# socom20/speech-cloner

Measured on AMD Instinct MI355X. Metric: mel frames/sec, higher is better.
Workload: dtype bf16; 1 GPU; full: STFT+mel front-end on batch 32 x 4 s @ 16 kHz (configs[1] input) -> 64 windows of 400 frames -> encoder (enc_14 weights) + decoder (hp/decoder_cfg_d.json sizes, random init), 64 windows per launch, independent steps pipelined over 10 HIP streams; batch=32, samples=64000, windows=64, model_dtype=bfloat16, streams=10, parallelism=utterance-sharded x1, no collective

## Files before the change

speech-cloner_amd/csrc/vc_common.h:

```cpp
#pragma once
#include <hip/hip_runtime.h>
#include <cstdarg>
#include <cstdio>
#include "vc_hip.h"

namespace vc {

char* last_error_buf();
int set_error(int code, const char* fmt, ...);

#define VC_HIP_CHECK(expr)                                                                   \
    do {                                                                                     \
        hipError_t _e = (expr);                                                              \
        if (_e != hipSuccess)                                                                \
            return vc::set_error(VC_ERR_HIP, "%s failed: %s (%s:%d)", #expr,                 \
                                 hipGetErrorString(_e), __FILE__, __LINE__);                 \
    } while (0)

#define VC_REQUIRE(cond, ...)                                                                \
    do {                                                                                     \
        if (!(cond)) return vc::set_error(VC_ERR_INVALID, __VA_ARGS__);                      \
    } while (0)

constexpr int WAVE = 64;

enum Option {
    OPT_BANK256 = 0,
    OPT_BANK256_XCD,
    OPT_CONV256,
    OPT_CONV256_MINK,
    OPT_CONV256_WM,
    OPT_PROJ256,
    OPT_PROJ256_SPLIT,
    OPT_WGRAD_XCD,
    OPT_GRU_MFMA,
    OPT_FE_FUSED,
    OPT_FE_FUSED_SPIN,
    OPT_PRENET_LDS,
    OPT_GRU_TRAIN_RESIDENT,
    OPT_CBHG_FRONT_MI,
    OPT_GRU_F32_WIDE,
    OPT_F32_F16X3,
    OPT_GEMM16_SPLIT,
    OPT_COUNT
};
int opt(Option o);

hipError_t zero_async(void* d_p, size_t bytes, hipStream_t st);

#if defined(__HIPCC__)
template <int CTRL, int ROW_MASK>
__device__ __forceinline__ float dpp_move(float identity, float v) {
    return __int_as_float(__builtin_amdgcn_update_dpp(__float_as_int(identity), __float_as_int(v), CTRL, ROW_MASK, 0xF, false));
}
#define VC_WAVE_REDUCE(OP, ID)                                                                  \
    v = OP(v, dpp_move<0xB1, 0xF>(ID, v));                             \
    v = OP(v, dpp_move<0x4E, 0xF>(ID, v));                             \
    v = OP(v, dpp_move<0x141, 0xF>(ID, v));                                \
    v = OP(v, dpp_move<0x140, 0xF>(ID, v));          \
    v = OP(v, dpp_move<0x142, 0xA>(ID, v));                 \
    v = OP(v, dpp_move<0x143, 0xC>(ID, v));                 \
    return __int_as_float(__builtin_amdgcn_readlane(__float_as_int(v), 63));
__device__ __forceinline__ float vc_addf(float a, float b) { return a + b; }
__device__ __forceinline__ float wave_sum(float v) { VC_WAVE_REDUCE(vc_addf, 0.0f) }
__device__ __forceinline__ float wave_max(float v) { VC_WAVE_REDUCE(fmaxf, -3.402823466e38f) }
__device__ __forceinline__ float wave_max_inf(float v) { VC_WAVE_REDUCE(fmaxf, v) }
__device__ __forceinline__ float highway_gate(float hpre, float tpre, float x) {
    const float hv = fmaxf(hpre, 0.0f);
    const float e = __builtin_amdgcn_exp2f(tpre * -1.4426950408889634f);
    const float tv = __builtin_amdgcn_rcpf(1.0f + e);
    return fmaf(tv, hv - x, x);
}
__device__ __forceinline__ float wave_min(float v) { VC_WAVE_REDUCE(fminf, 3.402823466e38f) }
#undef VC_WAVE_REDUCE
struct ArgMax { float v; int idx; };
__device__ __forceinline__ ArgMax wave_argmax_low(float v, int idx) {
#pragma unroll
    for (int s = 32; s > 0; s >>= 1) {
        const float ov = __shfl_xor(v, s, 64);
        const int oi = __shfl_xor(idx, s, 64);
        if (ov > v || (ov == v && oi < idx)) { v = ov; idx = oi; }
    }
    return {v, idx};
}

template <bool SUM, int NW>
__device__ inline int block_scan_excl(int v, int* wtot, int& total) {
    const int lane = threadIdx.x & 63, wave = threadIdx.x >> 6;
    const int ident = SUM ? 0 : -1;
    int inc = v;
#pragma unroll
    for (int s = 1; s < 64; s <<= 1) {
        const int u = __shfl_up(inc, s, 64);
        if (lane >= s) inc = SUM ? inc + u : max(inc, u);
    }
    int excl = __shfl_up(inc, 1, 64);
    if (lane == 0) excl = ident;
    __syncthreads();
    if (lane == 63) wtot[wave] = inc;
    __syncthreads();
    int off = ident, all = ident;
    for (int w = 0; w < NW; ++w) {
        const int x = wtot[w];
        if (w < wave) off = SUM ? off + x : max(off, x);
        all = SUM ? all + x : max(all, x);
    }
    total = all;
    return SUM ? excl + off : max(excl, off);
}

__device__ __forceinline__ float power_db_to_amp(float P, float inv_norm) {
    return exp10f(0.05f * (fmaxf(0.0f, P) * inv_norm - 80.0f));
}
#endif

}
```

speech-cloner_amd/csrc/vc_gemm.hip:

```cpp
#include <hip/hip_runtime.h>

#include <cstdlib>
#include "vc_device.h"
#include "vc_bank256.h"
#include "vc_conv256.h"

using vc::f32x16, vc::f32x4, vc::bf16x8;

namespace {

constexpr int BN = 128;
constexpr int ROWB = 144;
constexpr int GEMM_THREADS = 256;
constexpr int lds_bytes(int MI) { return 2 * (64 * MI + BN) * ROWB; }

template <typename T> struct Tr;
template <> struct Tr<float> {
    static constexpr int VEC = 4, BK = 32;
    typedef f32x4 vec_t;
};
template <> struct Tr<__bf16> {
    static constexpr int VEC = 8, BK = 64;
    typedef bf16x8 vec_t;
};
// ... 15 lines not shown
    const void* R;
    int32_t ldr;
    void* C;
    int32_t ldc, out_f32;
    float drop_keep;
    unsigned long long drop_seed;
    int32_t sum_groups;
    KGroup g[VC_GEMM_MAX_GROUPS];
};

__device__ __forceinline__ bool drop_keep_elem(unsigned long long idx, unsigned long long seed, float keep) {
    unsigned long long x = idx + seed * 0x9E3779B97F4A7C15ull;
    x ^= x >> 30; x *= 0xBF58476D1CE4E5B9ull;
    x ^= x >> 27; x *= 0x94D049BB133111EBull;
    x ^= x >> 31;
    return (float)(unsigned)(x >> 40) < keep * 16777216.0f;
}

__device__ __forceinline__ float to_f32(float v) { return v; }
__device__ __forceinline__ float to_f32(__bf16 v) { return (float)v; }

template <typename T> __device__ __forceinline__ void store_out(void* C, size_t idx, float v, int out_f32) {
    if (out_f32) reinterpret_cast<float*>(C)[idx] = v;
    else reinterpret_cast<T*>(C)[idx] = (T)v;
}

__device__ __forceinline__ f32x4 pro_apply(f32x4 v, const float* sc, const float* sh, int c, int relu) {
#pragma unroll
    for (int e = 0; e < 4; ++e) {
        float x = v[e];
        if (sc) x = x * sc[c + e] + sh[c + e];
        if (relu) x = fmaxf(x, 0.0f);
        v[e] = x;
    }
    return v;
}
__device__ __forceinline__ bf16x8 pro_apply(bf16x8 v, const float* sc, const float* sh, int c, int relu) {
#pragma unroll
    for (int e = 0; e < 8; ++e) {
        float x = (float)v[e];
        if (sc) x = x * sc[c + e] + sh[c + e];
        if (relu) x = fmaxf(x, 0.0f);
        v[e] = (__bf16)x;
    }
    return v;
}
__device__ __forceinline__ f32x4 vmax(f32x4 a, f32x4 b) {
#pragma unroll
    for (int e = 0; e < 4; ++e) a[e] = fmaxf(a[e], b[e]);
    return a;
}
__device__ __forceinline__ bf16x8 vmax(bf16x8 a, bf16x8 b) {
#pragma unroll
    for (int e = 0; e < 8; ++e) a[e] = ((float)a[e] >= (float)b[e]) ? a[e] : b[e];
    return a;
}

template <typename T, int MI> struct Mma;

template <int MI> struct Mma<float, MI> {
    static __device__ __forceinline__ void slab(const char* As, const char* Bs, int wm, int wn, int lane,
                                                f32x16 (&acc)[MI][2]) {
        const int i = lane & 31, h = lane >> 5;
        const char* ap = As + (wm * 32 * MI + i) * ROWB + h * 16;
        const char* bp = Bs + (wn * 64 + i) * ROWB + h * 16;
#pragma unroll
        for (int p = 0; p < 4; ++p) {
            f32x4 av[MI], bv[2];
#pragma unroll
            for (int mi = 0; mi < MI; ++mi) av[mi] = *reinterpret_cast<const f32x4*>(ap + mi * 32 * ROWB + p * 32);
            bv[0] = *reinterpret_cast<const f32x4*>(bp + p * 32);
            bv[1] = *reinterpret_cast<const f32x4*>(bp + 32 * ROWB + p * 32);
#pragma unroll
            for (int q = 0; q < 4; ++q)
#pragma unroll
                for (int mi = 0; mi < MI; ++mi)
#pragma unroll
                    for (int ni = 0; ni < 2; ++ni)
                        acc[mi][ni] = __builtin_amdgcn_mfma_f32_32x32x2f32(av[mi][q], bv[ni][q], acc[mi][ni], 0, 0, 0);
        }
    }
};

template <int MI> struct Mma<__bf16, MI> {
    static __device__ __forceinline__ void slab(const char* As, const char* Bs, int wm, int wn, int lane,
                                                f32x16 (&acc)[MI][2]) {
        const int i = lane & 31, h = lane >> 5;
        const char* ap = As + (wm * 32 * MI + i) * ROWB + h * 16;
        const char* bp = Bs + (wn * 64 + i) * ROWB + h * 16;
#pragma unroll
        for (int s = 0; s < 4; ++s) {
            bf16x8 av[MI], bv[2];
#pragma unroll
            for (int mi = 0; mi < MI; ++mi) av[mi] = *reinterpret_cast<const bf16x8*>(ap + mi * 32 * ROWB + s * 32);
            bv[0] = *reinterpret_cast<const bf16x8*>(bp + s * 32);
            bv[1] = *reinterpret_cast<const bf16x8*>(bp + 32 * ROWB + s * 32);
#pragma unroll
            for (int mi = 0; mi < MI; ++mi)
#pragma unroll
                for (int ni = 0; ni < 2; ++ni)
                    acc[mi][ni] = __builtin_amdgcn_mfma_f32_32x32x16_bf16(av[mi], bv[ni], acc[mi][ni], 0, 0, 0);
        }
    }
};


struct EpiCoef { float s[2], b[2]; };
__device__ __forceinline__ EpiCoef epilogue_coef(const KArgs& a, const KGroup& grp, int n0, int wn, int lane) {
    EpiCoef c;
#pragma unroll
    for (int ni = 0; ni < 2; ++ni) {
        const int oc = grp.c_off + min(n0 + wn * 64 + ni * 32 + (lane & 31), a.N - 1);
        c.s[ni] = a.epi_scale ? a.epi_scale[oc] : 1.0f;
        c.b[ni] = a.epi_shift ? a.epi_shift[oc] : 0.0f;
    }
    return c;
}

template <typename T, int MI>
__device__ __forceinline__ void epilogue_tile(const KArgs& a, const KGroup& grp, char* smem, const f32x16 (&acc)[MI][2],
                                              const EpiCoef& coef, int m0, int n0, int row_w, int wn, int lane, int tid) {
    constexpr int BM = 64 * MI;
    const bool f32o = a.out_f32 || sizeof(T) == 4;
    const int es = f32o ? 4 : 2;
    const int pitch = 128 * es + 16;
    const int i = lane & 31, h = lane >> 5;
#pragma unroll
    for (int ni = 0; ni < 2; ++ni) {
        const int lcol = wn * 64 + ni * 32 + i;
        const int gn = min(n0 + lcol, a.N - 1);
        const int oc = grp.c_off + gn;
        const float s = coef.s[ni], b = coef.b[ni];
#pragma unroll
        for (int mi = 0; mi < MI; ++mi) {
#pragma unroll
            for (int r = 0; r < 16; ++r) {
                const int lrow = row_w + mi * 32 + (r & 3) + 8 * (r >> 2) + 4 * h;
                const int gm = min(m0 + lrow, a.M - 1);
                float v = vc::act_fn(acc[mi][ni][r] * s + b, a.act);
                if (a.drop_keep > 0.0f)
                    v = drop_keep_elem((unsigned long long)gm * a.ldc + oc, a.drop_seed, a.drop_keep) ? v / a.drop_keep : 0.0f;
                if (a.R) v += to_f32(reinterpret_cast<const T*>(a.R)[(size_t)gm * a.ldr + gn]);
                char* dst = smem + lrow * pitch + lcol * es;
                if (f32o) *reinterpret_cast<float*>(dst) = v;
                else *reinterpret_cast<__bf16*>(dst) = (__bf16)v;
            }
        }
    }
    __syncthreads();
    const int chunk = 16 / es;
    const int cpr = 128 / chunk;
    char* C = reinterpret_cast<char*>(a.C);
    const bool vec_ok = ((reinterpret_cast<uintptr_t>(C) & 15) == 0) && ((a.ldc * es) % 16 == 0) &&
                        (((grp.c_off + n0) * es) % 16 == 0);
    for (int idx = tid; idx < BM * cpr; idx += GEMM_THREADS) {
        const int row = idx / cpr, ch = idx - row * cpr;
        const int gm = m0 + row, gn0 = n0 + ch * chunk;
        if (gm >= a.M || gn0 >= a.N) continue;
        const char* src = smem + row * pitch + ch * 16;
        char* dst = C + ((size_t)gm * a.ldc + grp.c_off + gn0) * es;
        if (vec_ok && gn0 + chunk <= a.N) {
            *reinterpret_cast<f32x4*>(dst) = *reinterpret_cast<const f32x4*>(src);
        } else {
            const int n = min(chunk, a.N - gn0);
            for (int e = 0; e < n; ++e) {
                if (f32o) reinterpret_cast<float*>(dst)[e] = reinterpret_cast<const float*>(src)[e];
                else reinterpret_cast<unsigned short*>(dst)[e] = reinterpret_cast<const unsigned short*>(src)[e];
            }
        }
    }
}

template <typename T, int MODE, int MI, int PRO>
__global__ void __launch_bounds__(GEMM_THREADS, 2)
gemm_kernel(KArgs a) {
    typedef typename Tr<T>::vec_t vec_t;
    constexpr int VEC = Tr<T>::VEC, BK = Tr<T>::BK;
    constexpr int BM = 64 * MI, AP = 2 * MI;
    constexpr int A_BYTES = BM * ROWB, B_BYTES = BN * ROWB, BUF_BYTES = A_BYTES + B_BYTES;
    extern __shared__ __attribute__((aligned(16))) char smem[];

    const int tid = threadIdx.x, lane = tid & 63, wid = tid >> 6;
    const int wm = wid >> 1, wn = wid & 1;
    const KGroup grp = a.g[a.n_groups - 1 - (int)blockIdx.y];
    const int ntn = (a.N + BN - 1) / BN;
    const int mt = blockIdx.x / ntn, nt = blockIdx.x - mt * ntn;
    const int m0 = mt * BM, n0 = nt * BN;
    const int K = grp.K, Cin = a.Cin, Tn = a.T;
    const int nk = (K + BK - 1) / BK;
    const T* X = reinterpret_cast<const T*>(a.X);
    const T* Bt = reinterpret_cast<const T*>(grp.Bt);

    const int sc = tid & 7, sr = tid >> 3;
    const T* a_row[AP];
    int a_t[AP];
    bool a_ok[AP], b_ok[4];
    const T* b_row[4];
#pragma unroll
    for (int p = 0; p < AP; ++p) {
        const int m = m0 + sr + 32 * p;
        a_ok[p] = m < a.M;
        const int mm = min(m, a.M - 1);
        a_t[p] = mm % Tn;
        a_row[p] = X + (size_t)mm * a.ldx;
    }
#pragma unroll
    for (int p = 0; p < 4; ++p) {
        const int n = n0 + sr + 32 * p;
        b_ok[p] = n < a.N;
        b_row[p] = Bt + (size_t)min(n, a.N - 1) * K;
    }
    const int pad_l = grp.pad_l, ldx = a.ldx;
    const bool pool = PRO >= 1 && a.pro_pool != 0;
    const bool nonneg = a.pro_pool == 2 || a.pro_relu;

    vec_t ra[AP], ra2[PRO >= 1 ? AP : 1], rb[4];
    unsigned okbits = 0;
    int st_c = 0;
    int g_kk = sc * VEC, g_j = 0, g_c = sc * VEC;
    if (grp.taps > 1) { g_j = g_c / Cin; g_c -= g_j * Cin; }
    auto gload = [&]() {
        const bool kok = g_kk < K;
        const int j = kok ? g_j : 0, c = kok ? g_c : 0, kb = kok ? g_kk : 0;
        const int dj = j - pad_l;
        unsigned bits = 0;
#pragma unroll
        for (int p = 0; p < AP; ++p) {
            const int tt = a_t[p] + dj;
            const bool ok = kok && a_ok[p] && tt >= 0 && tt < Tn;
            const T* ptr = a_row[p] + (ok ? dj * ldx : 0) + c;
            ra[p] = *reinterpret_cast<const vec_t*>(ptr);
            if (PRO >= 1) {
                const T* ptr2 = ptr + ((pool && ok && tt + 1 < Tn) ? ldx : 0);
                ra2[p] = *reinterpret_cast<const vec_t*>(ptr2);
            }
            bits |= (ok ? 1u : 0u) << p;
        }
#pragma unroll
        for (int p = 0; p < 4; ++p) {
            rb[p] = *reinterpret_cast<const vec_t*>(b_row[p] + kb);
            bits |= ((kok && b_ok[p]) ? 1u : 0u) << (8 + p);
        }
        okbits = bits;
        st_c = c;
        g_kk += BK;
        g_c += BK;
        if (grp.taps > 1)
            while (g_c >= Cin) { g_c -= Cin; ++g_j; }
    };
    auto lstore = [&](int buf) {
        char* As = smem + buf * BUF_BYTES;
        char* Bs = As + A_BYTES;
        const vec_t zero = {};
#pragma unroll
        for (int p = 0; p < AP; ++p) {
            vec_t v = ra[p];
            if (PRO == 2) v = pro_apply(v, a.pro_scale, a.pro_shift, st_c, a.pro_relu);
            if (PRO >= 1) {
                vec_t v2 = ra2[p];
                if (PRO == 2) v2 = pro_apply(v2, a.pro_scale, a.pro_shift, st_c, a.pro_relu);
                if (pool) v = nonneg ? vc::max_nonneg(v, v2) : vmax(v, v2);
            }
            *reinterpret_cast<vec_t*>(As + (sr + 32 * p) * ROWB + sc * 16) = ((okbits >> p) & 1u) ? v : zero;
        }
#pragma unroll
        for (int p = 0; p < 4; ++p)
            *reinterpret_cast<vec_t*>(Bs + (sr + 32 * p) * ROWB + sc * 16) = ((okbits >> (8 + p)) & 1u) ? rb[p] : zero;
    };

    f32x16 acc[MI][2];
#pragma unroll
    for (int mi = 0; mi < MI; ++mi)
#pragma unroll
        for (int ni = 0; ni < 2; ++ni)
#pragma unroll
            for (int r = 0; r < 16; ++r) acc[mi][ni][r] = 0.0f;

    const EpiCoef coef = (MODE == VC_GEMM_PLAIN) ? epilogue_coef(a, grp, n0, wn, lane) : EpiCoef{};
    gload();
    lstore(0);
    __syncthreads();
    for (int kt = 0; kt < nk; ++kt) {
        const bool more = kt + 1 < nk;
        if (more) gload();
        const char* As = smem + (kt & 1) * BUF_BYTES;
        Mma<T, MI>::slab(As, As + A_BYTES, wm, wn, lane, acc);
        if (more) lstore((kt + 1) & 1);
        __syncthreads();
    }

    const int i = lane & 31, h = lane >> 5;
    if (MODE == VC_GEMM_PLAIN) {
        epilogue_tile<T, MI>(a, grp, smem, acc, coef, m0, n0, wm * 32 * MI, wn, lane, tid);
    } else {
        const int hc = (n0 + wn * 64) / 2 + i;
        const int Hn = Cin;
        if (hc < Hn) {
            const int gnH = n0 + wn * 64 + i, gnT = gnH + 32;
            const float bH = a.epi_shift ? a.epi_shift[gnH] : 0.0f;
            const float bT = a.epi_shift ? a.epi_shift[gnT] : 0.0f;
#pragma unroll
            for (int mi = 0; mi < MI; ++mi) {
#pragma unroll
                for (int r = 0; r < 16; ++r) {
                    const int gm = m0 + wm * 32 * MI + mi * 32 + (r & 3) + 8 * (r >> 2) + 4 * h;
                    if (gm >= a.M) continue;
                    const float xv = to_f32(X[(size_t)gm * a.ldx + hc]);
                    store_out<T>(a.C, (size_t)gm * a.ldc + hc, vc::highway_gate(acc[mi][0][r] + bH, acc[mi][1][r] + bT, xv), a.out_f32);
                }
            }
        }
    }
}


constexpr int CONV_MAX_TAPS = 32;
constexpr int CROWB = ROWB;
constexpr int conv_lds_bytes() {
    return (128 + CONV_MAX_TAPS - 1) * CROWB + 2 * BN * CROWB > 128 * 528 ? (128 + CONV_MAX_TAPS - 1) * CROWB + 2 * BN * CROWB : 128 * 528;
}
__device__ __forceinline__ int swz(int row, int chunk) { return row * CROWB + (chunk << 4); }

template <typename T, int PRO>
__global__ void __launch_bounds__(GEMM_THREADS, 2)
conv_kernel(KArgs a) {
    typedef typename Tr<T>::vec_t vec_t;
    constexpr int VEC = Tr<T>::VEC, BK = Tr<T>::BK;
    constexpr int BM = 128, MI = 2;
    constexpr int A_BYTES = (BM + CONV_MAX_TAPS - 1) * CROWB, B_BYTES = BN * CROWB;
    constexpr int NAP = 5;
    extern __shared__ __attribute__((aligned(16))) char smem[];
    char* const As = smem;
    char* const Bs0 = smem + A_BYTES;

    const int tid = threadIdx.x, lane = tid & 63, wid = tid >> 6;
    const int wm = wid >> 1, wn = wid & 1;
    const int ntn = (a.N + BN - 1) / BN;
    const int mt = blockIdx.x / ntn, nt = blockIdx.x - mt * ntn;
    const int m0 = mt * BM, n0 = nt * BN;
    const int Cin = a.Cin, Tn = a.T, ldx = a.ldx;
    const int ncs = Cin / BK;
    const int li = lane & 31, lh = lane >> 5;
    f32x16 acc[MI][2];
#pragma unroll
    for (int mi = 0; mi < MI; ++mi)
#pragma unroll
        for (int ni = 0; ni < 2; ++ni)
#pragma unroll
            for (int r = 0; r < 16; ++r) acc[mi][ni][r] = 0.0f;
    const int g_lo = a.sum_groups ? 0 : a.n_groups - 1 - (int)blockIdx.y, g_hi = a.sum_groups ? a.n_groups : g_lo + 1;
    for (int gi = g_lo; gi < g_hi; ++gi) {
    if (a.sum_groups > 1 && min(gi, a.n_groups - 1 - gi) % a.sum_groups != (int)blockIdx.y) continue;
    const KGroup grp = a.g[gi];
    const int K = grp.K, taps = grp.taps, pad_l = grp.pad_l;
    const int NR = BM + taps - 1;
    const T* X = reinterpret_cast<const T*>(a.X) + (a.sum_groups ? grp.c_off : 0);
    const T* Bt = reinterpret_cast<const T*>(grp.Bt);
    const bool pool = PRO >= 1 && a.pro_pool != 0;
    const bool nonneg = a.pro_pool == 2 || a.pro_relu;

    const int sc = tid & 7, sr = tid >> 3;
    const T* a_row[NAP];
    const T* a_row2[NAP];
    bool a_in[NAP];
#pragma unroll
    for (int p = 0; p < NAP; ++p) {
        const int r = sr + 32 * p;
        a_in[p] = r < NR;
        const int g = min(max(m0 - pad_l + r, 0), a.M - 1);
        a_row[p] = X + (size_t)g * ldx + sc * VEC;
        const bool nxt = pool && (g % Tn) + 1 < Tn;
        a_row2[p] = a_row[p] + (nxt ? ldx : 0);
    }
    const T* b_row[4];
    bool b_ok[4];
#pragma unroll
    for (int p = 0; p < 4; ++p) {
        const int n = n0 + sr + 32 * p;
        b_ok[p] = n < a.N;
        b_row[p] = Bt + (size_t)min(n, a.N - 1) * K + sc * VEC;
    }
    int jlo[MI], jhi[MI];
#pragma unroll
    for (int mi = 0; mi < MI; ++mi) {
        const int m = min(m0 + wm * 64 + mi * 32 + li, a.M - 1);
        const int t = m % Tn;
        jlo[mi] = max(0, pad_l - t);
        jhi[mi] = min(taps, Tn - t + pad_l);
    }

    vec_t ra[NAP], ra2[PRO >= 1 ? NAP : 1];
    vec_t rbE[4], rbO[4];
    auto gloadA = [&](int cs) {
        const int c = cs * BK;
#pragma unroll
        for (int p = 0; p < NAP; ++p) {
            ra[p] = *reinterpret_cast<const vec_t*>(a_row[p] + c);
            if (PRO >= 1) ra2[p] = *reinterpret_cast<const vec_t*>(a_row2[p] + c);
        }
    };
    auto lstoreA = [&](int cs) {
        const int c = cs * BK + sc * VEC;
#pragma unroll
        for (int p = 0; p < NAP; ++p) {
            vec_t v = ra[p];
            if (PRO == 2) v = pro_apply(v, a.pro_scale, a.pro_shift, c, a.pro_relu);
            if (PRO >= 1) {
                vec_t v2 = ra2[p];
                if (PRO == 2) v2 = pro_apply(v2, a.pro_scale, a.pro_shift, c, a.pro_relu);
                if (pool) v = nonneg ? vc::max_nonneg(v, v2) : vmax(v, v2);
            }
            if (a_in[p]) *reinterpret_cast<vec_t*>(As + swz(sr + 32 * p, sc)) = v;
        }
    };
    int l_cs = 0, l_j = 0;
    auto gloadB = [&](vec_t* rb) {
        const int kb = l_j * Cin + l_cs * BK;
#pragma unroll
        for (int p = 0; p < 4; ++p) rb[p] = *reinterpret_cast<const vec_t*>(b_row[p] + kb);
        if (++l_j == taps) { l_j = 0; ++l_cs; }
    };
    const bool full_n = n0 + BN <= a.N;
    auto lstoreB = [&](int buf, const vec_t* rb) {
        char* Bs = Bs0 + buf * B_BYTES + sr * CROWB + sc * 16;
        const vec_t zero = {};
        if (full_n) {
#pragma unroll
            for (int p = 0; p < 4; ++p) *reinterpret_cast<vec_t*>(Bs + 32 * p * CROWB) = rb[p];
        } else {
#pragma unroll
            for (int p = 0; p < 4; ++p) *reinterpret_cast<vec_t*>(Bs + 32 * p * CROWB) = b_ok[p] ? rb[p] : zero;
        }
    };

    const int nit = ncs * taps;
    gloadA(0);
    gloadB(rbE);
    if (nit > 1) gloadB(rbO);
    lstoreA(0);
    lstoreB(0, rbE);
    __syncthreads();
    int cs = 0, j = 0;
    auto body = [&](int it, vec_t* rb_load, const vec_t* rb_store) {
        if (it + 2 < nit) gloadB(rb_load);
        const bool stageA = (j == 0) && (cs + 1 < ncs);
        if (stageA) gloadA(cs + 1);
        {
            const char* ap = As + (wm * 64 + li + j) * CROWB + lh * 16;
            const char* bp = Bs0 + (it & 1) * B_BYTES + (wn * 64 + li) * CROWB + lh * 16;
            const bool v0 = j >= jlo[0] && j < jhi[0], v1 = j >= jlo[1] && j < jhi[1];
            const vec_t zero = {};
            vec_t fa0[2], fa1[2], fb0[2], fb1[2];
            fa0[0] = *reinterpret_cast<const vec_t*>(ap);
            fa1[0] = *reinterpret_cast<const vec_t*>(ap + 32 * CROWB);
            fb0[0] = *reinterpret_cast<const vec_t*>(bp);
            fb1[0] = *reinterpret_cast<const vec_t*>(bp + 32 * CROWB);
#pragma unroll
            for (int s4 = 0; s4 < 4; ++s4) {
                const int cur = s4 & 1, nxt = cur ^ 1;
                if (s4 < 3) {
                    fa0[nxt] = *reinterpret_cast<const vec_t*>(ap + (s4 + 1) * 32);
                    fa1[nxt] = *reinterpret_cast<const vec_t*>(ap + 32 * CROWB + (s4 + 1) * 32);
                    fb0[nxt] = *reinterpret_cast<const vec_t*>(bp + (s4 + 1) * 32);
                    fb1[nxt] = *reinterpret_cast<const vec_t*>(bp + 32 * CROWB + (s4 + 1) * 32);
                }
                const vec_t av0 = v0 ? fa0[cur] : zero;
                const vec_t av1 = v1 ? fa1[cur] : zero;
                const vec_t bv0 = fb0[cur], bv1 = fb1[cur];
                if constexpr (sizeof(T) == 2) {
                    acc[0][0] = __builtin_amdgcn_mfma_f32_32x32x16_bf16(av0, bv0, acc[0][0], 0, 0, 0);
                    acc[0][1] = __builtin_amdgcn_mfma_f32_32x32x16_bf16(av0, bv1, acc[0][1], 0, 0, 0);
                    acc[1][0] = __builtin_amdgcn_mfma_f32_32x32x16_bf16(av1, bv0, acc[1][0], 0, 0, 0);
                    acc[1][1] = __builtin_amdgcn_mfma_f32_32x32x16_bf16(av1, bv1, acc[1][1], 0, 0, 0);
                } else {
#pragma unroll
                    for (int q = 0; q < 4; ++q) {
                        acc[0][0] = __builtin_amdgcn_mfma_f32_32x32x2f32(av0[q], bv0[q], acc[0][0], 0, 0, 0);
                        acc[0][1] = __builtin_amdgcn_mfma_f32_32x32x2f32(av0[q], bv1[q], acc[0][1], 0, 0, 0);
                        acc[1][0] = __builtin_amdgcn_mfma_f32_32x32x2f32(av1[q], bv0[q], acc[1][0], 0, 0, 0);
                        acc[1][1] = __builtin_amdgcn_mfma_f32_32x32x2f32(av1[q], bv1[q], acc[1][1], 0, 0, 0);
                    }
                }
            }
        }
        if (j == taps - 1 && cs + 1 < ncs) {
            __syncthreads();
            lstoreA(cs + 1);
        }
        if (it + 1 < nit) lstoreB((it + 1) & 1, rb_store);
        __syncthreads();
        if (++j == taps) { j = 0; ++cs; }
    };
    for (int it = 0; it < nit; it += 2) {
        body(it, rbE, rbO);
        if (it + 1 < nit) body(it + 1, rbO, rbE);
    }
    }

    KGroup og = a.g[g_lo];
    if (a.sum_groups) og.c_off = 0;
    if (a.sum_groups > 1) {
        float* C = reinterpret_cast<float*>(a.C);
#pragma unroll
        for (int mi = 0; mi < MI; ++mi)
#pragma unroll
            for (int ni = 0; ni < 2; ++ni) {
                const int gn = n0 + wn * 64 + ni * 32 + li;
#pragma unroll
                for (int r = 0; r < 16; ++r) {
                    const int gm = m0 + wm * 64 + mi * 32 + (r & 3) + 8 * (r >> 2) + 4 * lh;
                    if (gm < a.M && gn < a.N) unsafeAtomicAdd(C + (size_t)gm * a.ldc + gn, acc[mi][ni][r]);
                }
            }
        return;
    }
    const EpiCoef coef = epilogue_coef(a, og, n0, wn, lane);
    epilogue_tile<T, MI>(a, og, smem, acc, coef, m0, n0, wm * 64, wn, lane, tid);
}

template <typename T, int PRO> int launch_conv(const vc_gemm_desc* d, const KArgs& ka, hipStream_t st) {
    const int ntm = (d->M + 127) / 128, ntn = (d->N + BN - 1) / BN;
    if (int rc = vc::allow_dynamic_lds<conv_kernel<T, PRO>>(conv_lds_bytes())) return rc;
    hipLaunchKernelGGL((conv_kernel<T, PRO>), dim3(ntm * ntn, d->sum_groups ? d->sum_groups : d->n_groups), dim3(GEMM_THREADS), conv_lds_bytes(), st, ka);
    VC_HIP_CHECK(hipGetLastError());
    return VC_OK;
}


struct WGroup {
    const void* dYT;
    void* dW;
    int32_t N, taps, shift0, ldw;
};
struct WArgs {
    const void* XT;
    int32_t ldxt, ldyt, Cin, M, T, n_groups;
    int32_t splits;
    int32_t xcd_tiles;
    WGroup g[VC_GEMM_MAX_GROUPS];
};

typedef float f32x4u __attribute__((ext_vector_type(4), aligned(4)));

__global__ void __launch_bounds__(GEMM_THREADS, 2)
wgrad_kernel(WArgs a) {
    constexpr int MI = 2, BK = 32, BM = 128;
    constexpr int A_BYTES = BM * ROWB, B_BYTES = BN * ROWB, BUF_BYTES = A_BYTES + B_BYTES;
    extern __shared__ __attribute__((aligned(16))) char smem[];
    const int tid = threadIdx.x, lane = tid & 63, wid = tid >> 6;
    const int wm = wid >> 1, wn = wid & 1;
    int gsel, tile, zsplit;
    if (a.xcd_tiles > 0) {
        const int xcd = blockIdx.x & 7;
        int slot = blockIdx.x >> 3;
        zsplit = slot / a.xcd_tiles;
        slot -= zsplit * a.xcd_tiles;
        gsel = -1; tile = 0;
        for (int gi = 0; gi < a.n_groups; ++gi) {
            const int r16 = gi & 15;
            if ((r16 < 8 ? r16 : 15 - r16) != xcd) continue;
            const WGroup& gg = a.g[a.n_groups - 1 - gi];
            const int tg = ((gg.taps * a.Cin + BM - 1) / BM) * ((gg.N + BN - 1) / BN);
            if (slot < tg) { gsel = a.n_groups - 1 - gi; tile = slot; break; }
            slot -= tg;
        }
        if (gsel < 0) return;
    } else {
        gsel = a.n_groups - 1 - (int)blockIdx.y;
        tile = blockIdx.x;
        zsplit = blockIdx.z;
    }
    const WGroup grp = a.g[gsel];
    const int R = grp.taps * a.Cin;
    const int ntn = (grp.N + BN - 1) / BN, ntr = (R + BM - 1) / BM;
    if (tile >= ntr * ntn) return;
    const int rt = tile / ntn, nt = tile - rt * ntn;
    const int r0 = rt * BM, n0 = nt * BN;
    const int Tn = a.T, M = a.M;
    const int nk_all = (M + BK - 1) / BK;
    const int per = (nk_all + a.splits - 1) / a.splits;
    const int k_lo = zsplit * per, k_hi = min(nk_all, k_lo + per);
    const int nk = k_hi - k_lo;
    if (nk <= 0) return;
    const float* XT = reinterpret_cast<const float*>(a.XT);
    const float* YT = reinterpret_cast<const float*>(grp.dYT);

    const int sc = tid & 7, sr = tid >> 3;
    const float* a_base[4];
    const float* b_base[4];
    int a_dj[4];
    bool a_ok[4], b_ok[4];
#pragma unroll
    for (int p = 0; p < 4; ++p) {
        const int r = r0 + sr + 32 * p;
        a_ok[p] = r < R;
        const int rr = min(r, R - 1);
        const int j = rr / a.Cin, c = rr - j * a.Cin;
        a_dj[p] = j + grp.shift0;
        a_base[p] = XT + (size_t)c * a.ldxt + a_dj[p] + sc * 4;
        const int n = n0 + sr + 32 * p;
        b_ok[p] = n < grp.N;
        b_base[p] = YT + (size_t)min(n, grp.N - 1) * a.ldyt + sc * 4;
    }
    f32x4 ra[4], rb[4];
    int g_m = k_lo * BK;
    int st_m = 0;
    auto gload = [&]() {
#pragma unroll
        for (int p = 0; p < 4; ++p) {
            ra[p] = *reinterpret_cast<const f32x4u*>(a_base[p] + g_m);
            rb[p] = *reinterpret_cast<const f32x4u*>(b_base[p] + g_m);
// ... 314 lines not shown
```

speech-cloner_amd/csrc/vc_highway.hip:

```cpp
#include "vc_device.h"

using vc::f32x16, vc::f32x4, vc::bf16x8, vc::bf16x4;

namespace {

constexpr int HW_BM = 128;
constexpr int HW_MAX_LAYERS = 8;
constexpr int HW_RING = 4;

struct HwChainArgs {
    const __bf16* X;
    __bf16* Y;
    int32_t M, ldx, ldy, n_layers;
    const __bf16* W[HW_MAX_LAYERS];
    const float* bias[HW_MAX_LAYERS];
    const __bf16* PW;
    const float* Pbias;
    float* P;
    int32_t NP, ldp;
};

template <int H>
__device__ __forceinline__ void hw_tile(const bf16x8* pw, const bf16x8* next, const char* xrow, int lh, int x15,
                                        bf16x8 (&ring)[HW_RING][2], f32x16 (&acc)[4][2]) {
    constexpr int KS = H / 16, RB = 2 * H;
#pragma unroll
    for (int i = 0; i < 4; ++i)
#pragma unroll
        for (int c = 0; c < 2; ++c)
#pragma unroll
            for (int r = 0; r < 16; ++r) acc[i][c][r] = 0.0f;
    bf16x8 xf[2][4];
#pragma unroll
    for (int i = 0; i < 4; ++i) xf[0][i] = *reinterpret_cast<const bf16x8*>(xrow + i * 32 * RB + ((lh ^ x15) << 4));
#pragma unroll 1
    for (int s0 = 0; s0 < KS; s0 += HW_RING) {
        const bf16x8* src = (s0 + HW_RING < KS) ? pw + (size_t)(s0 + HW_RING) * 128 : next;
#pragma unroll
        for (int u = 0; u < HW_RING; ++u) {
            const int s = s0 + u, cb = u & 1;
            if (s + 1 < KS) {
#pragma unroll
                for (int i = 0; i < 4; ++i)
                    xf[cb ^ 1][i] = *reinterpret_cast<const bf16x8*>(xrow + i * 32 * RB + (((2 * (s + 1) + lh) ^ x15) << 4));
            }
            const bf16x8 w0 = ring[u][0], w1 = ring[u][1];
            if (src) {
                ring[u][0] = src[u * 128];
                ring[u][1] = src[u * 128 + 64];
            }
#pragma unroll
            for (int i = 0; i < 4; ++i) {
                acc[i][0] = __builtin_amdgcn_mfma_f32_32x32x16_bf16(w0, xf[cb][i], acc[i][0], 0, 0, 0);
                acc[i][1] = __builtin_amdgcn_mfma_f32_32x32x16_bf16(w1, xf[cb][i], acc[i][1], 0, 0, 0);
            }
        }
    }
}

template <int H>
__global__ void __launch_bounds__(2 * H, H == 256 ? 1 : 2)
highway_chain_kernel(HwChainArgs a) {
    constexpr int NT = 2 * H, KS = H / 16, RB = 2 * H, NS = H / 8;
    extern __shared__ __attribute__((aligned(16))) char smem[];
    const int tid = threadIdx.x, lane = tid & 63;
    const int w = __builtin_amdgcn_readfirstlane(tid >> 6);
    const int li = lane & 31, lh = lane >> 5, x15 = li & 15;
    const int m0 = blockIdx.x * HW_BM;

    for (int idx = tid; idx < HW_BM * NS; idx += NT) {
        const int row = idx / NS, slot = idx - row * NS;
        const int gm = min(m0 + row, a.M - 1);
        const bf16x8 v = *reinterpret_cast<const bf16x8*>(a.X + (size_t)gm * a.ldx + slot * 8);
        *reinterpret_cast<bf16x8*>(smem + row * RB + ((slot ^ (row & 15)) << 4)) = v;
    }

    float* bias_s = reinterpret_cast<float*>(smem + 2 * HW_BM * RB);
    for (int idx = tid; idx < a.n_layers * 2 * H; idx += NT) {
        const int l = idx / (2 * H);
        bias_s[idx] = a.bias[l][idx - l * 2 * H];
    }

    bf16x8 wr[HW_RING][2];
    auto wptr = [&](int layer, int s) {
        return reinterpret_cast<const bf16x8*>(a.W[layer]) + ((size_t)(w * KS + s) * 2) * 64 + lane;
    };
    if (a.n_layers > 0) {
#pragma unroll
        for (int s = 0; s < HW_RING; ++s) {
            const bf16x8* p = wptr(0, s);
            wr[s][0] = p[0];
            wr[s][1] = p[64];
        }
    }
    __syncthreads();

    for (int layer = 0; layer < a.n_layers; ++layer) {
        const char* cur = smem + (layer & 1) * (HW_BM * RB);
        char* nxt = smem + ((layer & 1) ^ 1) * (HW_BM * RB);
        const bool more = layer + 1 < a.n_layers;
        f32x16 acc[4][2];
        const bf16x8* nextw = more ? wptr(layer + 1, 0) : (a.PW && w < a.NP / 64 ? reinterpret_cast<const bf16x8*>(a.PW) + ((size_t)w * KS * 2) * 64 + lane : nullptr);
        hw_tile<H>(wptr(layer, 0), nextw, cur + li * RB, lh, x15, wr, acc);
        f32x4 bH[4], bT[4];
#pragma unroll
        for (int q = 0; q < 4; ++q) {
            bH[q] = *reinterpret_cast<const f32x4*>(bias_s + layer * 2 * H + w * 64 + 8 * q + 4 * lh);
            bT[q] = *reinterpret_cast<const f32x4*>(bias_s + layer * 2 * H + w * 64 + 32 + 8 * q + 4 * lh);
        }
#pragma unroll
        for (int i = 0; i < 4; ++i) {
#pragma unroll
            for (int q = 0; q < 4; ++q) {
                const int off = (i * 32 + li) * RB + (((4 * w + q) ^ x15) << 4) + lh * 8;
                const bf16x4 xin = *reinterpret_cast<const bf16x4*>(cur + off);
                bf16x4 o;
#pragma unroll
                for (int e = 0; e < 4; ++e) {
                    o[e] = (__bf16)vc::highway_gate(acc[i][0][4 * q + e] + bH[q][e], acc[i][1][4 * q + e] + bT[q][e], (float)xin[e]);
                }
                *reinterpret_cast<bf16x4*>(nxt + off) = o;
            }
        }
        __syncthreads();
    }

    const char* fin = smem + (a.n_layers & 1) * (HW_BM * RB);
    if (a.PW) {
        constexpr int NW = 2 * H / 64;
        const int ngroups = a.NP / 64;
        const char* xrow = fin + li * RB;
        char* const stg = smem + ((a.n_layers & 1) ^ 1) * (HW_BM * RB) + w * 8192;
        static_assert((2 * H / 64) * 8192 <= HW_BM * 2 * H, "a 32 x 64 float32 sub-tile per wave fits the idle buffer");
        if (a.n_layers == 0 && w < ngroups) {
            const bf16x8* p0 = reinterpret_cast<const bf16x8*>(a.PW) + ((size_t)w * KS * 2) * 64 + lane;
#pragma unroll
            for (int s = 0; s < HW_RING; ++s) { wr[s][0] = p0[s * 128]; wr[s][1] = p0[s * 128 + 64]; }
        }
        for (int grp = w; grp < ngroups; grp += NW) {
            const bf16x8* pw = reinterpret_cast<const bf16x8*>(a.PW) + ((size_t)grp * KS * 2) * 64 + lane;
            const bf16x8* nextw = (grp + NW < ngroups) ? pw + (size_t)NW * KS * 128 : nullptr;
            f32x16 acc[4][2];
            hw_tile<H>(pw, nextw, xrow, lh, x15, wr, acc);
#pragma unroll
            for (int c = 0; c < 2; ++c)
#pragma unroll
                for (int q = 0; q < 4; ++q) {
                    const f32x4 bb = *reinterpret_cast<const f32x4*>(a.Pbias + grp * 64 + c * 32 + 8 * q + 4 * lh);
#pragma unroll
                    for (int i = 0; i < 4; ++i)
#pragma unroll
                        for (int e = 0; e < 4; ++e) acc[i][c][4 * q + e] += bb[e];
                }
#pragma unroll
            for (int i = 0; i < 4; ++i) {
#pragma unroll
                for (int c = 0; c < 2; ++c)
#pragma unroll
                    for (int q = 0; q < 4; ++q) {
                        f32x4 o;
#pragma unroll
                        for (int e = 0; e < 4; ++e) o[e] = acc[i][c][4 * q + e];
                        *reinterpret_cast<f32x4*>(stg + li * 256 + (((c * 8 + 2 * q + lh) ^ x15) << 4)) = o;
                    }
#pragma unroll 2
                for (int j = 0; j < 8; ++j) {
                    const int row = j * 4 + (lane >> 4), ch = lane & 15;
                    const f32x4 v = *reinterpret_cast<const f32x4*>(stg + row * 256 + ((ch ^ (row & 15)) << 4));
                    const int gm = m0 + i * 32 + row;
                    if (gm < a.M) *reinterpret_cast<f32x4*>(a.P + (size_t)gm * a.ldp + grp * 64 + ch * 4) = v;
                }
            }
        }
    }
    if (a.Y == nullptr) return;
    for (int idx = tid; idx < HW_BM * NS; idx += NT) {
        const int row = idx / NS, slot = idx - row * NS;
        const int gm = m0 + row;
        if (gm < a.M)
            *reinterpret_cast<bf16x8*>(a.Y + (size_t)gm * a.ldy + slot * 8) =
                *reinterpret_cast<const bf16x8*>(fin + row * RB + ((slot ^ (row & 15)) << 4));
    }
}

template <int H> int launch_chain(const HwChainArgs& a, hipStream_t st) {
    constexpr int LDS = 2 * HW_BM * 2 * H + HW_MAX_LAYERS * 2 * H * 4;
    if (int rc = vc::allow_dynamic_lds<highway_chain_kernel<H>>(LDS)) return rc;
    hipLaunchKernelGGL(highway_chain_kernel<H>, dim3((a.M + HW_BM - 1) / HW_BM), dim3(2 * H), LDS, st, a);
    VC_HIP_CHECK(hipGetLastError());
    return VC_OK;
}

__global__ void __launch_bounds__(256)
highway_pack_kernel(const __bf16* Bt, int ncols, int H, __bf16* packed) {
    const int KS = H / 16, total = (ncols / 64) * KS * 2 * 64 * 8;
    for (int idx = blockIdx.x * 256 + threadIdx.x; idx < total; idx += gridDim.x * 256) {
        int r = idx;
        const int j = r & 7; r >>= 3;
        const int lane = r & 63; r >>= 6;
        const int c = r & 1; r >>= 1;
        const int s = r % KS;
        const int w = r / KS;
        packed[idx] = Bt[(size_t)(w * 64 + c * 32 + (lane & 31)) * H + s * 16 + (lane >> 5) * 8 + j];
    }
}

}

extern "C" {

int vc_highway_pack(const void* d_Bt, int32_t n_cols, int32_t H, void* d_packed, void* stream) {
    VC_REQUIRE(d_Bt && d_packed && (H == 128 || H == 256) && n_cols > 0 && n_cols % 64 == 0,
               "vc_highway_pack: H must be 128 or 256 and n_cols a multiple of 64");
    hipLaunchKernelGGL(highway_pack_kernel, dim3(128), dim3(256), 0, static_cast<hipStream_t>(stream),
                       static_cast<const __bf16*>(d_Bt), n_cols, H, static_cast<__bf16*>(d_packed));
    VC_HIP_CHECK(hipGetLastError());
    return VC_OK;
}

int vc_highway_chain(const void* d_X, int32_t M, int32_t H, int32_t ldx, int32_t n_layers, const void* const* d_packed,
                     const float* const* d_bias, void* d_Y, int32_t ldy, const void* d_proj_packed,
                     const float* d_proj_bias, int32_t n_proj, float* d_P, int32_t ldp, void* stream) {
    VC_REQUIRE(d_X && d_packed && d_bias && (d_Y || d_proj_packed), "vc_highway_chain: NULL argument");
    if (d_proj_packed)
        VC_REQUIRE(d_proj_bias && d_P && n_proj > 0 && n_proj % 64 == 0 && ldp >= n_proj && ldp % 4 == 0 &&
                       ((reinterpret_cast<uintptr_t>(d_proj_packed) | reinterpret_cast<uintptr_t>(d_proj_bias) |
                         reinterpret_cast<uintptr_t>(d_P)) & 15) == 0,
                   "vc_highway_chain: projection tail needs bias, output, n_proj %% 64 == 0, 16-byte aligned operands");
    VC_REQUIRE(H == 128 || H == 256, "vc_highway_chain: H must be 128 or 256 (got %d)", H);
    VC_REQUIRE(M > 0 && n_layers >= 0 && n_layers <= HW_MAX_LAYERS, "vc_highway_chain: bad M / n_layers");
    VC_REQUIRE(ldx >= H && ldx % 8 == 0 && (!d_Y || (ldy >= H && ldy % 8 == 0)), "vc_highway_chain: ldx / ldy must be multiples of 8 and >= H");
    VC_REQUIRE(((reinterpret_cast<uintptr_t>(d_X) | reinterpret_cast<uintptr_t>(d_Y)) & 15) == 0, "vc_highway_chain: X / Y must be 16-byte aligned");
    HwChainArgs a;
    a.X = static_cast<const __bf16*>(d_X); a.Y = static_cast<__bf16*>(d_Y);
    a.M = M; a.ldx = ldx; a.ldy = ldy; a.n_layers = n_layers;
    a.PW = static_cast<const __bf16*>(d_proj_packed); a.Pbias = d_proj_bias; a.P = d_P; a.NP = n_proj; a.ldp = ldp;
    for (int l = 0; l < n_layers; ++l) {
        VC_REQUIRE(d_packed[l] && d_bias[l] && (reinterpret_cast<uintptr_t>(d_packed[l]) & 15) == 0 &&
                       (reinterpret_cast<uintptr_t>(d_bias[l]) & 15) == 0, "vc_highway_chain: layer %d operands NULL or misaligned", l);
        a.W[l] = static_cast<const __bf16*>(d_packed[l]);
        a.bias[l] = d_bias[l];
    }
    hipStream_t st = static_cast<hipStream_t>(stream);
    return H == 256 ? launch_chain<256>(a, st) : launch_chain<128>(a, st);
}

}
```

Before: 14.37 million frames/s.

## Switch highway chain to 16x16x32 MFMA tiles and pair-vectorize highway gate

The fused highway-chain kernel now computes its 128-row tile with 16x16x32 bf16 MFMAs instead of 32x32x16. This changes the weight fragment layout, the activation loads, the accumulator shapes, and the epilogue and projection-staging indexing, and the weight prefetch ring shrinks from 4 to 2 steps of 4 fragments each. A two-wide vector highway_gate2 is added and used both in this kernel and in the GEMM highway epilogue, aiming to emit packed float ops. The smaller MFMA shape trades more instructions for different register pressure and latency, and the GEMM epilogue now does a clamped extra load of X per row pair.

```diff
diff --git a/speech-cloner_amd/csrc/vc_common.h b/speech-cloner_amd/csrc/vc_common.h
--- a/speech-cloner_amd/csrc/vc_common.h
+++ b/speech-cloner_amd/csrc/vc_common.h
@@ -71,6 +71,14 @@
     const float tv = __builtin_amdgcn_rcpf(1.0f + e);
     return fmaf(tv, hv - x, x);
 }
+typedef float f32x2 __attribute__((ext_vector_type(2)));
+__device__ __forceinline__ f32x2 highway_gate2(f32x2 hpre, f32x2 tpre, f32x2 x) {
+    const f32x2 hv = {fmaxf(hpre[0], 0.0f), fmaxf(hpre[1], 0.0f)};
+    const f32x2 s = tpre * -1.4426950408889634f;
+    const f32x2 d = 1.0f + f32x2{__builtin_amdgcn_exp2f(s[0]), __builtin_amdgcn_exp2f(s[1])};
+    const f32x2 tv = {__builtin_amdgcn_rcpf(d[0]), __builtin_amdgcn_rcpf(d[1])};
+    return __builtin_elementwise_fma(tv, hv - x, x);
+}
 __device__ __forceinline__ float wave_min(float v) { VC_WAVE_REDUCE(fminf, 3.402823466e38f) }
 #undef VC_WAVE_REDUCE
 struct ArgMax { float v; int idx; };
diff --git a/speech-cloner_amd/csrc/vc_gemm.hip b/speech-cloner_amd/csrc/vc_gemm.hip
--- a/speech-cloner_amd/csrc/vc_gemm.hip
+++ b/speech-cloner_amd/csrc/vc_gemm.hip
@@ -341,11 +341,15 @@
 #pragma unroll
             for (int mi = 0; mi < MI; ++mi) {
 #pragma unroll
-                for (int r = 0; r < 16; ++r) {
+                for (int r = 0; r < 16; r += 2) {
                     const int gm = m0 + wm * 32 * MI + mi * 32 + (r & 3) + 8 * (r >> 2) + 4 * h;
                     if (gm >= a.M) continue;
-                    const float xv = to_f32(X[(size_t)gm * a.ldx + hc]);
-                    store_out<T>(a.C, (size_t)gm * a.ldc + hc, vc::highway_gate(acc[mi][0][r] + bH, acc[mi][1][r] + bT, xv), a.out_f32);
+                    const int gm1 = min(gm + 1, a.M - 1);
+                    const vc::f32x2 xv = {to_f32(X[(size_t)gm * a.ldx + hc]), to_f32(X[(size_t)gm1 * a.ldx + hc])};
+                    const vc::f32x2 g = vc::highway_gate2(vc::f32x2{acc[mi][0][r], acc[mi][0][r + 1]} + bH,
+                                                          vc::f32x2{acc[mi][1][r], acc[mi][1][r + 1]} + bT, xv);
+                    store_out<T>(a.C, (size_t)gm * a.ldc + hc, g[0], a.out_f32);
+                    if (gm + 1 < a.M) store_out<T>(a.C, (size_t)(gm + 1) * a.ldc + hc, g[1], a.out_f32);
                 }
             }
         }
diff --git a/speech-cloner_amd/csrc/vc_highway.hip b/speech-cloner_amd/csrc/vc_highway.hip
--- a/speech-cloner_amd/csrc/vc_highway.hip
+++ b/speech-cloner_amd/csrc/vc_highway.hip
@@ -1,12 +1,12 @@
 #include "vc_device.h"
 
-using vc::f32x16, vc::f32x4, vc::bf16x8, vc::bf16x4;
+using vc::f32x4, vc::f32x2, vc::bf16x8, vc::bf16x4;
 
 namespace {
 
 constexpr int HW_BM = 128;
 constexpr int HW_MAX_LAYERS = 8;
-constexpr int HW_RING = 4;
+constexpr int HW_RING = 2;
 
 struct HwChainArgs {
     const __bf16* X;
@@ -20,39 +20,48 @@
     int32_t NP, ldp;
 };
 
+__device__ __forceinline__ int hw_lane_off(int lane) { return (lane >> 5) * 128 + ((lane >> 4) & 1) * 32 + (lane & 15); }
+constexpr int hw_frag_off(int c) { return (c >> 1) * 64 + (c & 1) * 16; }
+constexpr int HW_STEP = 256;
+
 template <int H>
-__device__ __forceinline__ void hw_tile(const bf16x8* pw, const bf16x8* next, const char* xrow, int lh, int x15,
-                                        bf16x8 (&ring)[HW_RING][2], f32x16 (&acc)[4][2]) {
-    constexpr int KS = H / 16, RB = 2 * H;
-#pragma unroll
-    for (int i = 0; i < 4; ++i)
-#pragma unroll
-        for (int c = 0; c < 2; ++c)
-#pragma unroll
-            for (int r = 0; r < 16; ++r) acc[i][c][r] = 0.0f;
+__device__ __forceinline__ void hw_tile(const bf16x8* pw, const bf16x8* next, const char* xrow, int lq, int x15,
+                                        bf16x8 (&ring)[HW_RING][4], f32x4 (&acc)[8][4]) {
+    constexpr int KS = H / 32, RB = 2 * H;
+    static_assert(KS % HW_RING == 0, "whole rings per tile");
+#pragma unroll
+    for (int i = 0; i < 8; ++i)
+#pragma unroll
+        for (int c = 0; c < 4; ++c) acc[i][c] = f32x4{0.0f, 0.0f, 0.0f, 0.0f};
     bf16x8 xf[2][4];
 #pragma unroll
-    for (int i = 0; i < 4; ++i) xf[0][i] = *reinterpret_cast<const bf16x8*>(xrow + i * 32 * RB + ((lh ^ x15) << 4));
+    for (int i = 0; i < 4; ++i) xf[0][i] = *reinterpret_cast<const bf16x8*>(xrow + i * 16 * RB + ((lq ^ x15) << 4));
 #pragma unroll 1
     for (int s0 = 0; s0 < KS; s0 += HW_RING) {
-        const bf16x8* src = (s0 + HW_RING < KS) ? pw + (size_t)(s0 + HW_RING) * 128 : next;
+        const bf16x8* src = (s0 + HW_RING < KS) ? pw + (size_t)(s0 + HW_RING) * HW_STEP : next;
 #pragma unroll
         for (int u = 0; u < HW_RING; ++u) {
-            const int s = s0 + u, cb = u & 1;
-            if (s + 1 < KS) {
+            const int s = s0 + u;
+            bf16x8 wf[4];
+#pragma unroll
+            for (int c = 0; c < 4; ++c) wf[c] = ring[u][c];
+            if (src) {
+#pragma unroll
+                for (int c = 0; c < 4; ++c) ring[u][c] = src[u * HW_STEP + hw_frag_off(c)];
+            }
+#pragma unroll
+            for (int h = 0; h < 2; ++h) {
+                if (h == 0 || s + 1 < KS) {
+                    const int sn = s + h, hn = h ^ 1;
+#pragma unroll
+                    for (int i = 0; i < 4; ++i)
+                        xf[hn][i] = *reinterpret_cast<const bf16x8*>(xrow + (4 * hn + i) * 16 * RB + (((4 * sn + lq) ^ x15) << 4));
+                }
 #pragma unroll
                 for (int i = 0; i < 4; ++i)
-                    xf[cb ^ 1][i] = *reinterpret_cast<const bf16x8*>(xrow + i * 32 * RB + (((2 * (s + 1) + lh) ^ x15) << 4));
-            }
-            const bf16x8 w0 = ring[u][0], w1 = ring[u][1];
-            if (src) {
-                ring[u][0] = src[u * 128];
-                ring[u][1] = src[u * 128 + 64];
-            }
-#pragma unroll
-            for (int i = 0; i < 4; ++i) {
-                acc[i][0] = __builtin_amdgcn_mfma_f32_32x32x16_bf16(w0, xf[cb][i], acc[i][0], 0, 0, 0);
-                acc[i][1] = __builtin_amdgcn_mfma_f32_32x32x16_bf16(w1, xf[cb][i], acc[i][1], 0, 0, 0);
+#pragma unroll
+                    for (int c = 0; c < 4; ++c)
+                        acc[4 * h + i][c] = __builtin_amdgcn_mfma_f32_16x16x32_bf16(wf[c], xf[h][i], acc[4 * h + i][c], 0, 0, 0);
             }
         }
     }
@@ -61,11 +70,12 @@
 template <int H>
 __global__ void __launch_bounds__(2 * H, H == 256 ? 1 : 2)
 highway_chain_kernel(HwChainArgs a) {
-    constexpr int NT = 2 * H, KS = H / 16, RB = 2 * H, NS = H / 8;
+    constexpr int NT = 2 * H, KS16 = H / 16, RB = 2 * H, NS = H / 8;
+    constexpr int GRP = KS16 * 128;
     extern __shared__ __attribute__((aligned(16))) char smem[];
     const int tid = threadIdx.x, lane = tid & 63;
     const int w = __builtin_amdgcn_readfirstlane(tid >> 6);
-    const int li = lane & 31, lh = lane >> 5, x15 = li & 15;
+    const int x15 = lane & 15, lq = lane >> 4;
     const int m0 = blockIdx.x * HW_BM;
 
     for (int idx = tid; idx < HW_BM * NS; idx += NT) {
@@ -81,17 +91,20 @@
         bias_s[idx] = a.bias[l][idx - l * 2 * H];
     }
 
-    bf16x8 wr[HW_RING][2];
-    auto wptr = [&](int layer, int s) {
-        return reinterpret_cast<const bf16x8*>(a.W[layer]) + ((size_t)(w * KS + s) * 2) * 64 + lane;
+    bf16x8 wr[HW_RING][4];
+    const int loff = hw_lane_off(lane);
+    auto wptr = [&](int layer) {
+        return reinterpret_cast<const bf16x8*>(a.W[layer]) + (size_t)w * GRP + loff;
+    };
+    auto pptr = [&](int grp) {
+        return reinterpret_cast<const bf16x8*>(a.PW) + (size_t)grp * GRP + loff;
     };
     if (a.n_layers > 0) {
-#pragma unroll
-        for (int s = 0; s < HW_RING; ++s) {
-            const bf16x8* p = wptr(0, s);
-            wr[s][0] = p[0];
-            wr[s][1] = p[64];
-        }
+        const bf16x8* p = wptr(0);
+#pragma unroll
+        for (int s = 0; s < HW_RING; ++s)
+#pragma unroll
+            for (int c = 0; c < 4; ++c) wr[s][c] = p[s * HW_STEP + hw_frag_off(c)];
     }
     __syncthreads();
 
@@ -99,25 +112,29 @@
         const char* cur = smem + (layer & 1) * (HW_BM * RB);
         char* nxt = smem + ((layer & 1) ^ 1) * (HW_BM * RB);
         const bool more = layer + 1 < a.n_layers;
-        f32x16 acc[4][2];
-        const bf16x8* nextw = more ? wptr(layer + 1, 0) : (a.PW && w < a.NP / 64 ? reinterpret_cast<const bf16x8*>(a.PW) + ((size_t)w * KS * 2) * 64 + lane : nullptr);
-        hw_tile<H>(wptr(layer, 0), nextw, cur + li * RB, lh, x15, wr, acc);
-        f32x4 bH[4], bT[4];
-#pragma unroll
-        for (int q = 0; q < 4; ++q) {
-            bH[q] = *reinterpret_cast<const f32x4*>(bias_s + layer * 2 * H + w * 64 + 8 * q + 4 * lh);
-            bT[q] = *reinterpret_cast<const f32x4*>(bias_s + layer * 2 * H + w * 64 + 32 + 8 * q + 4 * lh);
-        }
-#pragma unroll
-        for (int i = 0; i < 4; ++i) {
-#pragma unroll
-            for (int q = 0; q < 4; ++q) {
-                const int off = (i * 32 + li) * RB + (((4 * w + q) ^ x15) << 4) + lh * 8;
+        f32x4 acc[8][4];
+        const bf16x8* nextw = more ? wptr(layer + 1) : (a.PW && w < a.NP / 64 ? pptr(w) : nullptr);
+        hw_tile<H>(wptr(layer), nextw, cur + x15 * RB, lq, x15, wr, acc);
+        f32x4 bH[2], bT[2];
+#pragma unroll
+        for (int c = 0; c < 2; ++c) {
+            bH[c] = *reinterpret_cast<const f32x4*>(bias_s + layer * 2 * H + w * 64 + 16 * c + 4 * lq);
+            bT[c] = *reinterpret_cast<const f32x4*>(bias_s + layer * 2 * H + w * 64 + 32 + 16 * c + 4 * lq);
+        }
+#pragma unroll
+        for (int i = 0; i < 8; ++i) {
+#pragma unroll
+            for (int c = 0; c < 2; ++c) {
+                const int off = (i * 16 + x15) * RB + (((4 * w + 2 * c + (lq >> 1)) ^ x15) << 4) + (lq & 1) * 8;
                 const bf16x4 xin = *reinterpret_cast<const bf16x4*>(cur + off);
                 bf16x4 o;
 #pragma unroll
-                for (int e = 0; e < 4; ++e) {
-                    o[e] = (__bf16)vc::highway_gate(acc[i][0][4 * q + e] + bH[q][e], acc[i][1][4 * q + e] + bT[q][e], (float)xin[e]);
+                for (int e = 0; e < 4; e += 2) {
+                    const f32x2 hp = f32x2{acc[i][c][e], acc[i][c][e + 1]} + f32x2{bH[c][e], bH[c][e + 1]};
+                    const f32x2 tp = f32x2{acc[i][c + 2][e], acc[i][c + 2][e + 1]} + f32x2{bT[c][e], bT[c][e + 1]};
+                    const f32x2 g = vc::highway_gate2(hp, tp, f32x2{(float)xin[e], (float)xin[e + 1]});
+                    o[e] = (__bf16)g[0];
+                    o[e + 1] = (__bf16)g[1];
                 }
                 *reinterpret_cast<bf16x4*>(nxt + off) = o;
             }
@@ -129,45 +146,39 @@
     if (a.PW) {
         constexpr int NW = 2 * H / 64;
         const int ngroups = a.NP / 64;
-        const char* xrow = fin + li * RB;
+        const char* xrow = fin + x15 * RB;
         char* const stg = smem + ((a.n_layers & 1) ^ 1) * (HW_BM * RB) + w * 8192;
         static_assert((2 * H / 64) * 8192 <= HW_BM * 2 * H, "a 32 x 64 float32 sub-tile per wave fits the idle buffer");
         if (a.n_layers == 0 && w < ngroups) {
-            const bf16x8* p0 = reinterpret_cast<const bf16x8*>(a.PW) + ((size_t)w * KS * 2) * 64 + lane;
-#pragma unroll
-            for (int s = 0; s < HW_RING; ++s) { wr[s][0] = p0[s * 128]; wr[s][1] = p0[s * 128 + 64]; }
+            const bf16x8* p0 = pptr(w);
+#pragma unroll
+            for (int s = 0; s < HW_RING; ++s)
+#pragma unroll
+                for (int c = 0; c < 4; ++c) wr[s][c] = p0[s * HW_STEP + hw_frag_off(c)];
         }
         for (int grp = w; grp < ngroups; grp += NW) {
-            const bf16x8* pw = reinterpret_cast<const bf16x8*>(a.PW) + ((size_t)grp * KS * 2) * 64 + lane;
-            const bf16x8* nextw = (grp + NW < ngroups) ? pw + (size_t)NW * KS * 128 : nullptr;
-            f32x16 acc[4][2];
-            hw_tile<H>(pw, nextw, xrow, lh, x15, wr, acc);
-#pragma unroll
-            for (int c = 0; c < 2; ++c)
-#pragma unroll
-                for (int q = 0; q < 4; ++q) {
-                    const f32x4 bb = *reinterpret_cast<const f32x4*>(a.Pbias + grp * 64 + c * 32 + 8 * q + 4 * lh);
-#pragma unroll
-                    for (int i = 0; i < 4; ++i)
-#pragma unroll
-                        for (int e = 0; e < 4; ++e) acc[i][c][4 * q + e] += bb[e];
-                }
-#pragma unroll
-            for (int i = 0; i < 4; ++i) {
-#pragma unroll
-                for (int c = 0; c < 2; ++c)
-#pragma unroll
-                    for (int q = 0; q < 4; ++q) {
-                        f32x4 o;
-#pragma unroll
-                        for (int e = 0; e < 4; ++e) o[e] = acc[i][c][4 * q + e];
-                        *reinterpret_cast<f32x4*>(stg + li * 256 + (((c * 8 + 2 * q + lh) ^ x15) << 4)) = o;
-                    }
+            const bf16x8* pw = pptr(grp);
+            const bf16x8* nextw = (grp + NW < ngroups) ? pw + (size_t)NW * GRP : nullptr;
+            f32x4 acc[8][4];
+            hw_tile<H>(pw, nextw, xrow, lq, x15, wr, acc);
+#pragma unroll
+            for (int c = 0; c < 4; ++c) {
+                const f32x4 bb = *reinterpret_cast<const f32x4*>(a.Pbias + grp * 64 + 16 * c + 4 * lq);
+#pragma unroll
+                for (int i = 0; i < 8; ++i) acc[i][c] += bb;
+            }
+#pragma unroll
+            for (int ip = 0; ip < 4; ++ip) {
+#pragma unroll
+                for (int t = 0; t < 2; ++t)
+#pragma unroll
+                    for (int c = 0; c < 4; ++c)
+                        *reinterpret_cast<f32x4*>(stg + (16 * t + x15) * 256 + (((4 * c + lq) ^ x15) << 4)) = acc[2 * ip + t][c];
 #pragma unroll 2
                 for (int j = 0; j < 8; ++j) {
                     const int row = j * 4 + (lane >> 4), ch = lane & 15;
                     const f32x4 v = *reinterpret_cast<const f32x4*>(stg + row * 256 + ((ch ^ (row & 15)) << 4));
-                    const int gm = m0 + i * 32 + row;
+                    const int gm = m0 + ip * 32 + row;
                     if (gm < a.M) *reinterpret_cast<f32x4*>(a.P + (size_t)gm * a.ldp + grp * 64 + ch * 4) = v;
                 }
             }
```

Result: no change. 14.41 million frames/s, median of 5 (+0.3%).
